# LanceZPF/loongx

Hardware: AMD Instinct MI355X
Metric: edited images/s @512x512, 28-step Flux denoise (higher is better)
Workload: dtype bf16

## Files before the change

### loongx_amd/csrc/rowops.hip

```cpp
#include "common.h"
#include <type_traits>

namespace {

struct LnLora { const uint16_t* A; float* T; int R, ldt, row0, rows; };

template <int NCH, bool LM = false, bool F16 = false>
__global__ __launch_bounds__(256, 3) void ln_modulate_kernel(const float* __restrict__ X, int ldx, const LnSegs segs, int mod_ld,
                                                          uint16_t* __restrict__ Y, int ldy, int M, int D, float eps, const LnLora lo = LnLora{},
                                                          int* __restrict__ f16_ovf = nullptr) {
  constexpr int RS = NCH * 256 + 32;
  __shared__ __attribute__((aligned(16))) uint16_t rows_s[LM ? 4 * RS : 8];
  __shared__ f32x4 red_s[LM ? 4 * 64 : 1];
  const int wave = threadIdx.x >> 6;
  const int row_l = blockIdx.x * 4 + wave;
  if constexpr (!LM) {
    if (row_l >= M) return;
  }
  const bool valid = row_l < M;
  auto phys = [&](int rl, int& sg_o, int& rin_o) {
    int sg = 0, acc_rows = 0;
    while (sg < segs.n - 1 && rl >= acc_rows + segs.n_rows[sg]) { acc_rows += segs.n_rows[sg]; ++sg; }
    sg_o = sg; rin_o = rl - acc_rows;
    return segs.row0[sg] + rin_o;
  };
  int sg, rin;
  const int row = phys(min(row_l, M - 1), sg, rin);
  bool wg_lora = false;
  if constexpr (LM) {
#pragma unroll
    for (int w = 0; w < 4; ++w) {
      const int rl = blockIdx.x * 4 + w;
      int s2, r2;
      const int pr = phys(min(rl, M - 1), s2, r2);
      wg_lora |= rl < M && pr >= lo.row0 && pr < lo.row0 + lo.rows;
    }
  }
  const float* shift = segs.shift[sg];
  const float* scale = segs.scale[sg];
  const int rows_per_batch = segs.rows_per_batch[sg];
  const int lane = threadIdx.x & 63;
  const float* xr = X + (size_t)row * ldx;
  f32x4 v[NCH];
  float s = 0.f;
#pragma unroll
  for (int i = 0; i < NCH; ++i) v[i] = *(const f32x4*)(xr + (i * 64 + lane) * 4);
  const int b = rin / rows_per_batch;
  const float* sh = shift + (size_t)b * mod_ld;
  const float* sc = scale + (size_t)b * mod_ld;
  f32x4 av[NCH], bv[NCH];
#pragma unroll
  for (int i = 0; i < NCH; ++i) {
    av[i] = *(const f32x4*)(sc + (i * 64 + lane) * 4);
    bv[i] = *(const f32x4*)(sh + (i * 64 + lane) * 4);
  }
#pragma unroll
  for (int i = 0; i < NCH; ++i) s += (v[i][0] + v[i][1]) + (v[i][2] + v[i][3]);
  const float mean = wave_total(s) / (float)D;
  float q = 0.f;
#pragma unroll
  for (int i = 0; i < NCH; ++i)
#pragma unroll
    for (int c = 0; c < 4; ++c) {
      const float d = v[i][c] - mean;
      q += d * d;
    }
  const float rstd = rsqrtf(wave_total(q) / (float)D + eps);
  uint16_t* yr = Y + (size_t)row * ldy;
  float f16_mx = 0.f;
#pragma unroll
  for (int i = 0; i < NCH; ++i) {
    const int col = (i * 64 + lane) * 4;
    float o[4];
#pragma unroll
    for (int c = 0; c < 4; ++c) o[c] = (v[i][c] - mean) * rstd * (1.0f + av[i][c]) + bv[i][c];
    u32x2 w;
    w[0] = pack_op16x2<F16>(o[0], o[1], f16_mx);
    w[1] = pack_op16x2<F16>(o[2], o[3], f16_mx);
    if (valid) *(u32x2*)(yr + col) = w;
    if constexpr (LM) {
      if (wg_lora) *(u32x2*)(rows_s + wave * RS + col) = w;
    }
  }
  if constexpr (LM) {
    if (wg_lora) {
      constexpr int NS = 2 * NCH, NB = NS >= 8 ? NS / 2 : NS;
      const int l15 = lane & 15, kq = lane >> 4;
      const uint16_t* ap = lo.A + (size_t)min(l15, lo.R - 1) * D + kq * 8;
      __builtin_amdgcn_sched_barrier(0);
      bf16x8 af[NB];
#pragma unroll
      for (int u = 0; u < NB; ++u) af[u] = *(const bf16x8*)(ap + (4 * u + wave) * 32);
      __syncthreads();
      f32x4 acc = {0.f, 0.f, 0.f, 0.f};
      const uint16_t* xp = rows_s + (l15 & 3) * RS + kq * 8;
      const bf16x8 zero = {};
#pragma unroll
      for (int u0 = 0; u0 < NS; u0 += NB) {
        if (u0 > 0) {
#pragma unroll
          for (int u = 0; u < NB; ++u) af[u] = *(const bf16x8*)(ap + (4 * (u0 + u) + wave) * 32);
        }
#pragma unroll
        for (int u = 0; u < NB; ++u) {
          bf16x8 xf = *(const bf16x8*)(xp + (4 * (u0 + u) + wave) * 32);
          xf = l15 < 4 ? xf : zero;
          if constexpr (F16) acc = __builtin_amdgcn_mfma_f32_16x16x32_f16(__builtin_bit_cast(f16x8, af[u]), __builtin_bit_cast(f16x8, xf), acc, 0, 0, 0);
          else acc = __builtin_amdgcn_mfma_f32_16x16x32_bf16(af[u], xf, acc, 0, 0, 0);
        }
      }
      red_s[wave * 64 + lane] = acc;
      __syncthreads();
      if (threadIdx.x < 64) {
        const int m = threadIdx.x >> 4, r = threadIdx.x & 15;
        const float* rp = (const float*)red_s + (m + 16 * (r >> 2)) * 4 + (r & 3);
        const float t = ((rp[0] + rp[256]) + rp[512]) + rp[768];
        const int rl = blockIdx.x * 4 + m;
        int s2, r2;
        const int pr = phys(min(rl, M - 1), s2, r2);
        if (rl < M && r < lo.R && pr >= lo.row0 && pr < lo.row0 + lo.rows) lo.T[(size_t)(pr - lo.row0) * lo.ldt + r] = t;
      }
    }
  }
  if constexpr (F16) report_f16_overflow(f16_mx, f16_ovf);
}

template <bool F16 = false>
__global__ __launch_bounds__(256) void ln_modulate_generic(const float* __restrict__ X, int ldx, const LnSegs segs, int mod_ld,
                                                           uint16_t* __restrict__ Y, int ldy, int M, int D, float eps, int* __restrict__ f16_ovf = nullptr) {
  int row = blockIdx.x * 4 + (threadIdx.x >> 6);
  if (row >= M) return;
  int sg = 0, acc_rows = 0;
  while (sg < segs.n - 1 && row >= acc_rows + segs.n_rows[sg]) { acc_rows += segs.n_rows[sg]; ++sg; }
  const int rin = row - acc_rows;
  row = segs.row0[sg] + rin;
  const float* shift = segs.shift[sg];
  const float* scale = segs.scale[sg];
  const int rows_per_batch = segs.rows_per_batch[sg];
  const int lane = threadIdx.x & 63;
  const float* xr = X + (size_t)row * ldx;
  float s = 0.f;
  for (int c = lane * 4; c < D; c += 256) {
    const f32x4 v = *(const f32x4*)(xr + c);
    s += (v[0] + v[1]) + (v[2] + v[3]);
  }
  const float mean = wave_sum(s) / (float)D;
  float q = 0.f;
  for (int c = lane * 4; c < D; c += 256) {
    const f32x4 v = *(const f32x4*)(xr + c);
#pragma unroll
    for (int k = 0; k < 4; ++k) q += (v[k] - mean) * (v[k] - mean);
  }
  const float rstd = rsqrtf(wave_sum(q) / (float)D + eps);
  const int b = rin / rows_per_batch;
  const float* sh = shift + (size_t)b * mod_ld;
  const float* sc = scale + (size_t)b * mod_ld;
  uint16_t* yr = Y + (size_t)row * ldy;
  float f16_mx = 0.f;
  for (int c = lane * 4; c < D; c += 256) {
    const f32x4 v = *(const f32x4*)(xr + c);
    const f32x4 a = *(const f32x4*)(sc + c);
    const f32x4 bsh = *(const f32x4*)(sh + c);
    float o[4];
#pragma unroll
    for (int k = 0; k < 4; ++k) o[k] = (v[k] - mean) * rstd * (1.0f + a[k]) + bsh[k];
    u32x2 w;
    w[0] = pack_op16x2<F16>(o[0], o[1], f16_mx);
    w[1] = pack_op16x2<F16>(o[2], o[3], f16_mx);
    *(u32x2*)(yr + c) = w;
  }
  if constexpr (F16) report_f16_overflow(f16_mx, f16_ovf);
}

__device__ __forceinline__ int vt_interleave(int key) {
  return (key & ~15) | (((key >> 2) & 1) << 3) | (((key >> 3) & 1) << 2) | (key & 3);
}

struct QkvSegs {
  int n;
  int row0[3], rows_per_batch[3], vt_pos0[3], tile0[4];
  const float* wq[3]; const float* wk[3]; const float* cos_tab[3]; const float* sin_tab[3];
};

__device__ __forceinline__ void unpack16x8(const u32x4 raw, float* x, bool in_f16) {
#pragma unroll
  for (int i = 0; i < 4; ++i) {
    if (in_f16) {
      x[2 * i] = (float)__builtin_bit_cast(_Float16, (uint16_t)(raw[i] & 0xffffu));
      x[2 * i + 1] = (float)__builtin_bit_cast(_Float16, (uint16_t)(raw[i] >> 16));
    } else {
      x[2 * i] = __uint_as_float(raw[i] << 16);
      x[2 * i + 1] = __uint_as_float(raw[i] & 0xffff0000u);
    }
  }
}
__device__ __forceinline__ u32x4 f16x8_to_bf16x8(const u32x4 raw) {
  float x[8];
  unpack16x8(raw, x, true);
  u32x4 o;
#pragma unroll
  for (int i = 0; i < 4; ++i) o[i] = pack_bf16x2(x[2 * i], x[2 * i + 1]);
  return o;
}

template <bool FAST, bool IN_F16 = false, bool KIMG = false>
__global__ __launch_bounds__(256) void qkv_prep_kernel(uint16_t* __restrict__ QKV, int ld, int q_col, int k_col, int v_col,
                                                       const QkvSegs segs, float eps, uint16_t* __restrict__ VT, int vt_ld, int H,
                                                       uint16_t* __restrict__ K2, int ldk2, int k2_col) {
  __shared__ uint16_t vt_s[64][128 + 8];
  int sg = 0;
  while (sg < segs.n - 1 && (int)blockIdx.x >= segs.tile0[sg + 1]) ++sg;
  const int p0 = ((int)blockIdx.x - segs.tile0[sg]) * 64;
  const int row0 = segs.row0[sg], rows_per_batch = segs.rows_per_batch[sg], vt_pos0 = segs.vt_pos0[sg];
  const float* __restrict__ wq = segs.wq[sg];
  const float* __restrict__ wk = segs.wk[sg];
  const float* __restrict__ cos_tab = segs.cos_tab[sg];
  const float* __restrict__ sin_tab = segs.sin_tab[sg];
  const int h = blockIdx.y;
  const int b = blockIdx.z;
  const int tid = threadIdx.x;
  const int sub = tid & 15;
  const int rloc = tid >> 4;
  const size_t rbase = (size_t)row0 + (size_t)b * rows_per_batch;
  if constexpr (FAST) {
    const f32x4 wq0 = *(const f32x4*)(wq + sub * 8), wq1 = *(const f32x4*)(wq + sub * 8 + 4);
    const f32x4 wk0 = *(const f32x4*)(wk + sub * 8), wk1 = *(const f32x4*)(wk + sub * 8 + 4);
#pragma unroll 1
    for (int half = 0; half < 2; ++half) {
      uint16_t* rowp[2];
      uint16_t* kdst[2];
      bool valid[2];
      u32x4 raw[2][3];
      f32x4 cs[2][4];
#pragma unroll
      for (int u = 0; u < 2; ++u) {
        const int p = p0 + (half * 2 + u) * 16 + rloc;
        valid[u] = p < rows_per_batch;
        const int pc = valid[u] ? p : 0;
        rowp[u] = QKV + (rbase + pc) * ld + h * 128 + sub * 8;
        kdst[u] = KIMG ? K2 + (rbase + pc) * ldk2 + k2_col + h * 128 + sub * 8 : rowp[u] + k_col;
        raw[u][0] = *(const u32x4*)(rowp[u] + q_col);
        raw[u][1] = *(const u32x4*)(rowp[u] + k_col);
        raw[u][2] = *(const u32x4*)(rowp[u] + v_col);
        const float* ct = cos_tab + (size_t)pc * 128 + sub * 8;
        const float* st = sin_tab + (size_t)pc * 128 + sub * 8;
        cs[u][0] = *(const f32x4*)ct; cs[u][1] = *(const f32x4*)(ct + 4);
        cs[u][2] = *(const f32x4*)st; cs[u][3] = *(const f32x4*)(st + 4);
      }
      __builtin_amdgcn_sched_barrier(0);
#pragma unroll
      for (int u = 0; u < 2; ++u) {
        u32x4 out[2];
#pragma unroll
        for (int which = 0; which < 2; ++which) {
          float x[8];
#pragma unroll
          for (int i = 0; i < 4; ++i) {
            x[2 * i] = __uint_as_float(raw[u][which][i] << 16);
            x[2 * i + 1] = __uint_as_float(raw[u][which][i] & 0xffff0000u);
          }
          float ss = 0.f;
#pragma unroll
          for (int i = 0; i < 8; ++i) ss += x[i] * x[i];
#pragma unroll
          for (int o = 8; o > 0; o >>= 1) ss += __shfl_xor(ss, o, 64);
          const float r = rsqrtf(ss * (1.0f / 128.0f) + eps);
          const f32x4 w0 = which ? wk0 : wq0, w1 = which ? wk1 : wq1;
#pragma unroll
          for (int i = 0; i < 4; ++i) { x[i] = x[i] * r * w0[i]; x[4 + i] = x[4 + i] * r * w1[i]; }
          float y[8];
#pragma unroll
          for (int i = 0; i < 4; ++i) {
            const float ce = i < 2 ? cs[u][0][2 * i] : cs[u][1][2 * i - 4], co = i < 2 ? cs[u][0][2 * i + 1] : cs[u][1][2 * i - 3];
            const float se = i < 2 ? cs[u][2][2 * i] : cs[u][3][2 * i - 4], so = i < 2 ? cs[u][2][2 * i + 1] : cs[u][3][2 * i - 3];
            y[2 * i] = x[2 * i] * ce - x[2 * i + 1] * se;
            y[2 * i + 1] = x[2 * i + 1] * co + x[2 * i] * so;
          }
#pragma unroll
          for (int i = 0; i < 4; ++i) out[which][i] = pack_bf16x2(y[2 * i], y[2 * i + 1]);
        }
        if (valid[u]) {
          *(u32x4*)(rowp[u] + q_col) = out[0];
          *(u32x4*)kdst[u] = out[1];
        }
        if (VT) *(u32x4*)&vt_s[(half * 2 + u) * 16 + rloc][sub * 8] = valid[u] ? raw[u][2] : u32x4{0u, 0u, 0u, 0u};
      }
    }
  } else {
#pragma unroll 1
  for (int pass = 0; pass < 4; ++pass) {
    const int p = p0 + pass * 16 + rloc;
    const bool valid = p < rows_per_batch;
    uint16_t* rowp = QKV + (rbase + (valid ? p : 0)) * ld + h * 128 + sub * 8;
    f32x4 c0 = {1.f, 1.f, 1.f, 1.f}, c1 = c0, s0 = {0.f, 0.f, 0.f, 0.f}, s1 = s0;
    if (cos_tab && valid) {
      const float* ct = cos_tab + (size_t)p * 128 + sub * 8;
      const float* st = sin_tab + (size_t)p * 128 + sub * 8;
      c0 = *(const f32x4*)ct; c1 = *(const f32x4*)(ct + 4);
      s0 = *(const f32x4*)st; s1 = *(const f32x4*)(st + 4);
    }
#pragma unroll
    for (int which = 0; which < 2; ++which) {
      const float* wn = which ? wk : wq;
      uint16_t* ptr = rowp + (which ? k_col : q_col);
      uint16_t* dst = ptr;
      if constexpr (KIMG) {
        if (which) dst = K2 + (rbase + (valid ? p : 0)) * ldk2 + k2_col + h * 128 + sub * 8;
      }
      u32x4 raw = {0u, 0u, 0u, 0u};
      if (valid) raw = *(const u32x4*)ptr;
      float x[8];
      unpack16x8(raw, x, IN_F16);
      if (wn) {
        float ss = 0.f;
#pragma unroll
        for (int i = 0; i < 8; ++i) ss += x[i] * x[i];
#pragma unroll
        for (int o = 8; o > 0; o >>= 1) ss += __shfl_xor(ss, o, 64);
        const float r = rsqrtf(ss * (1.0f / 128.0f) + eps);
        const f32x4 w0 = *(const f32x4*)(wn + sub * 8), w1 = *(const f32x4*)(wn + sub * 8 + 4);
#pragma unroll
        for (int i = 0; i < 4; ++i) { x[i] = x[i] * r * w0[i]; x[4 + i] = x[4 + i] * r * w1[i]; }
      }
      float y[8];
#pragma unroll
      for (int i = 0; i < 4; ++i) {
        const float ce = i < 2 ? c0[2 * i] : c1[2 * i - 4], co = i < 2 ? c0[2 * i + 1] : c1[2 * i - 3];
        const float se = i < 2 ? s0[2 * i] : s1[2 * i - 4], so = i < 2 ? s0[2 * i + 1] : s1[2 * i - 3];
        y[2 * i] = x[2 * i] * ce - x[2 * i + 1] * se;
        y[2 * i + 1] = x[2 * i + 1] * co + x[2 * i] * so;
      }
      if (valid) {
        u32x4 o;
#pragma unroll
        for (int i = 0; i < 4; ++i) o[i] = pack_bf16x2(y[2 * i], y[2 * i + 1]);
        *(u32x4*)dst = o;
      }
    }
    if (VT) {
      u32x4 raw = {0u, 0u, 0u, 0u};
      if (valid) raw = *(const u32x4*)(rowp + v_col);
      *(u32x4*)&vt_s[pass * 16 + rloc][sub * 8] = IN_F16 ? f16x8_to_bf16x8(raw) : raw;
    }
  }
  }
  if (!VT) return;
  __syncthreads();
  uint16_t* vtb = VT + ((size_t)(b * H + h) * 128) * vt_ld + vt_pos0 + p0;
  for (int item = tid; item < 128 * 8; item += 256) {
    const int d = item >> 3, g = item & 7;
    uint16_t e[8];
#pragma unroll
    for (int i = 0; i < 8; ++i) e[i] = vt_s[vt_interleave(g * 8 + i)][d];
    u32x4 o;
#pragma unroll
    for (int i = 0; i < 4; ++i) o[i] = (uint32_t)e[2 * i] | ((uint32_t)e[2 * i + 1] << 16);
    *(u32x4*)(vtb + (size_t)d * vt_ld + g * 8) = o;
  }
}

__device__ __forceinline__ float clamp_e4m3(float x) { return fminf(fmaxf(x, -448.f), 448.f); }
__device__ __forceinline__ uint32_t pack_fp8x4(float a, float b, float c, float d) {
  int w = __builtin_amdgcn_cvt_pk_fp8_f32(clamp_e4m3(a), clamp_e4m3(b), 0, false);
  w = __builtin_amdgcn_cvt_pk_fp8_f32(clamp_e4m3(c), clamp_e4m3(d), w, true);
  return (uint32_t)w;
}
__device__ __forceinline__ int vt8_key(int j) {
  const int g = j >> 5, p = j & 31;
  return (p >> 4) * 32 + 8 * ((p & 15) >> 2) + 4 * g + (p & 3);
}

template <bool IN_F16>
__global__ __launch_bounds__(256) void qkv_prep_fp8_kernel(const uint16_t* __restrict__ QKV, int ld, int q_col, int k_col, int v_col,
                                                           const QkvSegs segs, float eps, uint8_t* __restrict__ Q8,
                                                           uint8_t* __restrict__ K8, int ld8, uint8_t* __restrict__ VT8, int vt_ld,
                                                           int H, float q_scale, float k_scale, float v_scale) {
  __shared__ uint16_t vt_s[64][128 + 8];
  int sg = 0;
  while (sg < segs.n - 1 && (int)blockIdx.x >= segs.tile0[sg + 1]) ++sg;
  const int p0 = ((int)blockIdx.x - segs.tile0[sg]) * 64;
  const int row0 = segs.row0[sg], rows_per_batch = segs.rows_per_batch[sg], vt_pos0 = segs.vt_pos0[sg];
  const float* __restrict__ wq = segs.wq[sg];
  const float* __restrict__ wk = segs.wk[sg];
  const float* __restrict__ cos_tab = segs.cos_tab[sg];
  const float* __restrict__ sin_tab = segs.sin_tab[sg];
  const int h = blockIdx.y;
  const int b = blockIdx.z;
  const int tid = threadIdx.x;
  const int sub = tid & 15;
  const int rloc = tid >> 4;
  const size_t rbase = (size_t)row0 + (size_t)b * rows_per_batch;
#pragma unroll 1
  for (int pass = 0; pass < 4; ++pass) {
    const int p = p0 + pass * 16 + rloc;
    const bool valid = p < rows_per_batch;
    const size_t grow = rbase + (valid ? p : 0);
    const uint16_t* rowp = QKV + grow * ld + h * 128 + sub * 8;
    f32x4 c0 = {1.f, 1.f, 1.f, 1.f}, c1 = c0, s0 = {0.f, 0.f, 0.f, 0.f}, s1 = s0;
    if (cos_tab && valid) {
      const float* ct = cos_tab + (size_t)p * 128 + sub * 8;
      const float* st = sin_tab + (size_t)p * 128 + sub * 8;
      c0 = *(const f32x4*)ct; c1 = *(const f32x4*)(ct + 4);
      s0 = *(const f32x4*)st; s1 = *(const f32x4*)(st + 4);
    }
#pragma unroll
    for (int which = 0; which < 2; ++which) {
      const float* wn = which ? wk : wq;
      u32x4 raw = {0u, 0u, 0u, 0u};
      if (valid) raw = *(const u32x4*)(rowp + (which ? k_col : q_col));
      float x[8];
      unpack16x8(raw, x, IN_F16);
      if (wn) {
        float ss = 0.f;
#pragma unroll
        for (int i = 0; i < 8; ++i) ss += x[i] * x[i];
#pragma unroll
        for (int o = 8; o > 0; o >>= 1) ss += __shfl_xor(ss, o, 64);
        const float r = rsqrtf(ss * (1.0f / 128.0f) + eps);
        const f32x4 w0 = *(const f32x4*)(wn + sub * 8), w1 = *(const f32x4*)(wn + sub * 8 + 4);
#pragma unroll
        for (int i = 0; i < 4; ++i) { x[i] = x[i] * r * w0[i]; x[4 + i] = x[4 + i] * r * w1[i]; }
      }
      float y[8];
#pragma unroll
      for (int i = 0; i < 4; ++i) {
        const float ce = i < 2 ? c0[2 * i] : c1[2 * i - 4], co = i < 2 ? c0[2 * i + 1] : c1[2 * i - 3];
        const float se = i < 2 ? s0[2 * i] : s1[2 * i - 4], so = i < 2 ? s0[2 * i + 1] : s1[2 * i - 3];
        y[2 * i] = x[2 * i] * ce - x[2 * i + 1] * se;
        y[2 * i + 1] = x[2 * i + 1] * co + x[2 * i] * so;
      }
      if (valid) {
        const float sc = which ? k_scale : q_scale;
        u32x2 o;
        o[0] = pack_fp8x4(y[0] * sc, y[1] * sc, y[2] * sc, y[3] * sc);
        o[1] = pack_fp8x4(y[4] * sc, y[5] * sc, y[6] * sc, y[7] * sc);
        *(u32x2*)((which ? K8 : Q8) + grow * ld8 + h * 128 + sub * 8) = o;
      }
    }
    u32x4 raw = {0u, 0u, 0u, 0u};
    if (valid) raw = *(const u32x4*)(rowp + v_col);
    *(u32x4*)&vt_s[pass * 16 + rloc][sub * 8] = IN_F16 ? f16x8_to_bf16x8(raw) : raw;
  }
  __syncthreads();
  uint8_t* vtb = VT8 + ((size_t)(b * H + h) * 128) * vt_ld + vt_pos0 + p0;
  for (int item = tid; item < 128 * 4; item += 256) {
    const int d = item >> 2, c = item & 3;
    float e[16];
#pragma unroll
    for (int i = 0; i < 16; ++i) e[i] = __uint_as_float((uint32_t)vt_s[vt8_key(c * 16 + i)][d] << 16) * v_scale;
    u32x4 o;
#pragma unroll
    for (int i = 0; i < 4; ++i) o[i] = pack_fp8x4(e[4 * i], e[4 * i + 1], e[4 * i + 2], e[4 * i + 3]);
    *(u32x4*)(vtb + (size_t)d * vt_ld + c * 16) = o;
  }
}

struct LoraTerms {
  const uint16_t* X[4];
  const uint16_t* A[4];
  int ldx[4];
  int n;
};

template <bool F16 = false>
__global__ __launch_bounds__(512) void lora_down_mfma_kernel(const LoraTerms terms, float* __restrict__ T, int ldt, int M, int K, int R, int Ks,
                                                             int split_stride) {
  __shared__ f32x4 red[8][64];
  const int lane = threadIdx.x & 63, wave = threadIdx.x >> 6;
  const int m0 = blockIdx.x * 16;
  const int term = terms.n > 0 ? (int)blockIdx.y : 0;
  const uint16_t* __restrict__ X = terms.X[term];
  const uint16_t* __restrict__ A = terms.A[term];
  const int ldx = terms.ldx[term];
  const int kbeg = terms.n > 0 ? 0 : blockIdx.y * Ks, kend = terms.n > 0 ? K : min(K, kbeg + Ks);
  T += (size_t)blockIdx.y * split_stride;
  const int l15 = lane & 15, kq = lane >> 4;
  const uint16_t* xp = X + (size_t)min(m0 + l15, M - 1) * ldx + kq * 8;
  const uint16_t* ap = A + (size_t)min(l15, R - 1) * K + kq * 8;
  f32x4 acc = {0.f, 0.f, 0.f, 0.f};
  int k = kbeg + wave * 32;
  const bf16x8 zero = {};
  auto batch = [&](auto n_) {
    constexpr int NS = decltype(n_)::value;
    bf16x8 af[NS], xf[NS];
#pragma unroll
    for (int u = 0; u < NS; ++u) {
      const bool in = k + u * 256 < kend;
      af[u] = in ? *(const bf16x8*)(ap + k + u * 256) : zero;
      xf[u] = in ? *(const bf16x8*)(xp + k + u * 256) : zero;
    }
#pragma unroll
    for (int u = 0; u < NS; ++u) {
      if constexpr (F16) acc = __builtin_amdgcn_mfma_f32_16x16x32_f16(__builtin_bit_cast(f16x8, af[u]), __builtin_bit_cast(f16x8, xf[u]), acc, 0, 0, 0);
      else acc = __builtin_amdgcn_mfma_f32_16x16x32_bf16(af[u], xf[u], acc, 0, 0, 0);
    }
    k += NS * 256;
  };
  const int nsteps = k < kend ? (kend - k + 255) / 256 : 0;
  if (nsteps <= 4) batch(std::integral_constant<int, 4>{});
  else if (nsteps <= 8) batch(std::integral_constant<int, 8>{});
  else
    while (k < kend) batch(std::integral_constant<int, 16>{});
  red[wave][lane] = acc;
  __syncthreads();
  if (wave == 0) {
#pragma unroll
    for (int w = 1; w < 8; ++w) {
      const f32x4 o = red[w][lane];
      acc[0] += o[0]; acc[1] += o[1]; acc[2] += o[2]; acc[3] += o[3];
    }
    const int m = m0 + l15, r0 = 4 * kq;
    if (m < M && r0 < R) {
      float* tp = T + (size_t)m * ldt + r0;
      if (r0 + 4 <= R && (ldt & 3) == 0) *(f32x4*)tp = acc;
      else
        for (int j = 0; j < 4 && r0 + j < R; ++j) tp[j] = acc[j];
    }
  }
}

template <bool F16>
__global__ __launch_bounds__(512) void lora_down_wide_kernel(const uint16_t* __restrict__ X, int ldx, const uint16_t* __restrict__ A,
                                                             float* __restrict__ T, int ldt, int M, int K, int R, int Ks, int split_stride) {
  __shared__ f32x4 red[8][4][64];
  const int lane = threadIdx.x & 63, wave = threadIdx.x >> 6;
  const int m0 = blockIdx.x * 16, rz0 = blockIdx.z * 64;
  const int nt = min(4, (R - rz0 + 15) / 16);
  const int kbeg = blockIdx.y * Ks, kend = min(K, kbeg + Ks);
  T += (size_t)blockIdx.y * split_stride;
  const int l15 = lane & 15, kq = lane >> 4;
  const uint16_t* xp = X + (size_t)min(m0 + l15, M - 1) * ldx + kq * 8;
  const uint16_t* ap[4];
#pragma unroll
  for (int t = 0; t < 4; ++t) ap[t] = A + (size_t)min(rz0 + t * 16 + l15, R - 1) * K + kq * 8;
  f32x4 acc[4];
#pragma unroll
  for (int t = 0; t < 4; ++t) acc[t] = f32x4{0.f, 0.f, 0.f, 0.f};
  int k = kbeg + wave * 32;
  const bf16x8 zero = {};
  auto batch = [&](auto n_) {
    constexpr int NS = decltype(n_)::value;
    bf16x8 af[NS][4], xf[NS];
#pragma unroll
    for (int u = 0; u < NS; ++u) {
      const bool in = k + u * 256 < kend;
      xf[u] = in ? *(const bf16x8*)(xp + k + u * 256) : zero;
#pragma unroll
      for (int t = 0; t < 4; ++t) af[u][t] = (in && t < nt) ? *(const bf16x8*)(ap[t] + k + u * 256) : zero;
    }
#pragma unroll
    for (int u = 0; u < NS; ++u)
#pragma unroll
      for (int t = 0; t < 4; ++t)
        if (t < nt) {
          if constexpr (F16) acc[t] = __builtin_amdgcn_mfma_f32_16x16x32_f16(__builtin_bit_cast(f16x8, af[u][t]), __builtin_bit_cast(f16x8, xf[u]), acc[t], 0, 0, 0);
          else acc[t] = __builtin_amdgcn_mfma_f32_16x16x32_bf16(af[u][t], xf[u], acc[t], 0, 0, 0);
        }
    k += NS * 256;
  };
  const int nsteps = k < kend ? (kend - k + 255) / 256 : 0;
  if (nsteps <= 4) batch(std::integral_constant<int, 4>{});
  else
    while (k < kend) batch(std::integral_constant<int, 8>{});
#pragma unroll
  for (int t = 0; t < 4; ++t) red[wave][t][lane] = acc[t];
  __syncthreads();
  if (wave < nt) {
    f32x4 s = red[0][wave][lane];
#pragma unroll
    for (int w = 1; w < 8; ++w) {
      const f32x4 o = red[w][wave][lane];
      s[0] += o[0]; s[1] += o[1]; s[2] += o[2]; s[3] += o[3];
    }
    const int m = m0 + l15, r0 = rz0 + 16 * wave + 4 * kq;
    if (m < M && r0 < R) {
      float* tp = T + (size_t)m * ldt + r0;
      if (r0 + 4 <= R && (ldt & 3) == 0) *(f32x4*)tp = s;
      else
        for (int j = 0; j < 4 && r0 + j < R; ++j) tp[j] = s[j];
    }
  }
}

__device__ __forceinline__ float silu(float x) { return x / (1.0f + __expf(-x)); }

__global__ __launch_bounds__(256) void linear_skinny_kernel(const float* __restrict__ X, int ldx, const uint16_t* __restrict__ W,
                                                            int ldw, const float* __restrict__ bias, float* __restrict__ Y,
                                                            int ldy, int M, int N, int K, int act_in, int act_out, int accumulate) {
  const int wave = threadIdx.x >> 6, lane = threadIdx.x & 63;
  const int n0 = (blockIdx.x * 4 + wave) * 4;
  if (n0 >= N) return;
  const uint16_t* wr[4];
#pragma unroll
  for (int c = 0; c < 4; ++c) wr[c] = W + (size_t)min(n0 + c, N - 1) * ldw;
  for (int mb = 0; mb < M; mb += 4) {
    float acc[4][4];
#pragma unroll
    for (int i = 0; i < 4; ++i)
#pragma unroll
      for (int c = 0; c < 4; ++c) acc[i][c] = 0.f;
    for (int k = lane * 8; k < K; k += 512) {
      float wv[4][8];
#pragma unroll
      for (int c = 0; c < 4; ++c) {
        const u32x4 raw = *(const u32x4*)(wr[c] + k);
#pragma unroll
        for (int j = 0; j < 4; ++j) { wv[c][2 * j] = __uint_as_float(raw[j] << 16); wv[c][2 * j + 1] = __uint_as_float(raw[j] & 0xffff0000u); }
      }
#pragma unroll
      for (int i = 0; i < 4; ++i) {
        if (mb + i < M) {
          const float* xp = X + (size_t)(mb + i) * ldx + k;
          const f32x4 x0 = *(const f32x4*)xp, x1 = *(const f32x4*)(xp + 4);
          float xv[8] = {x0[0], x0[1], x0[2], x0[3], x1[0], x1[1], x1[2], x1[3]};
          if (act_in == 1) {
#pragma unroll
            for (int j = 0; j < 8; ++j) xv[j] = silu(xv[j]);
          }
#pragma unroll
          for (int c = 0; c < 4; ++c)
#pragma unroll
            for (int j = 0; j < 8; ++j) acc[i][c] = fmaf(xv[j], wv[c][j], acc[i][c]);
        }
      }
    }
#pragma unroll
    for (int i = 0; i < 4; ++i)
#pragma unroll
      for (int c = 0; c < 4; ++c) {
        float s = wave_sum(acc[i][c]);
        if (lane == 0 && mb + i < M && n0 + c < N) {
          if (bias) s += bias[n0 + c];
          if (act_out == 1) s = silu(s);
          float* yp = Y + (size_t)(mb + i) * ldy + n0 + c;
          *yp = accumulate ? (*yp + s) : s;
        }
      }
  }
}

__global__ void timestep_embed_kernel(const float* __restrict__ t, float* __restrict__ out, int B, int dim) {
  const int i = blockIdx.x * blockDim.x + threadIdx.x;
  const int half = dim / 2;
  if (i >= B * half) return;
  const int b = i / half, j = i % half;
  const float f = expf(-9.210340371976184f * (float)j / (float)half);
  const float a = t[b] * f;
  out[(size_t)b * dim + j] = cosf(a);
  out[(size_t)b * dim + half + j] = sinf(a);
}

__global__ void euler_kernel(float* __restrict__ x, const void* __restrict__ v, int v_bf16, float ds, size_t n) {
  const size_t stride = (size_t)gridDim.x * blockDim.x;
  for (size_t i = (size_t)blockIdx.x * blockDim.x + threadIdx.x; i < n; i += stride) {
    const float vv = v_bf16 ? bf16_to_f32(((const uint16_t*)v)[i]) : ((const float*)v)[i];
    x[i] = fmaf(ds, vv, x[i]);
  }
}

__global__ void convert_kernel(void* __restrict__ dst, int dst_bf16, const void* __restrict__ src, int src_bf16, size_t n) {
  const size_t stride = (size_t)gridDim.x * blockDim.x;
  for (size_t i = (size_t)blockIdx.x * blockDim.x + threadIdx.x; i < n; i += stride) {
    const float v = src_bf16 ? bf16_to_f32(((const uint16_t*)src)[i]) : ((const float*)src)[i];
    if (dst_bf16 == 2) {
      float mx = 0.f;
      ((uint16_t*)dst)[i] = (uint16_t)(pack_f16x2_sat(v, 0.f, mx) & 0xffffu);
    } else if (dst_bf16) ((uint16_t*)dst)[i] = f32_to_bf16(v);
    else ((float*)dst)[i] = v;
  }
}

}

static int ln_launch(const char* name, const float* X, int ldx, const lx_ln_seg* seg, int n_seg, int mod_ld, void* Y, int ldy, int D, float eps,
                     void* stream, const LnLora* lora = nullptr, bool f16 = false, int* f16_ovf = nullptr) {
  LX_CHECK_ARG(seg && n_seg >= 1 && n_seg <= 3, "%s: 1..3 segments", name);
  if (f16) LX_CHECK_ARG(((uintptr_t)f16_ovf & 3) == 0, "%s: f16_ovf must be 4-byte aligned", name);
  LnSegs segs;
  const int M = lx_ln_segs("lx_ln_modulate", seg, n_seg, segs);
  if (M < 0) return M;
  LX_CHECK_ARG(X && Y, "lx_ln_modulate: NULL operand");
  LX_CHECK_ARG(D > 0 && D % 4 == 0 && D <= 16384, "lx_ln_modulate: D=%d must be a multiple of 4 and <= 16384", D);
  LX_CHECK_ARG(ldx % 4 == 0 && ldy % 4 == 0 && mod_ld % 4 == 0, "lx_ln_modulate: ldx/ldy/mod_ld must be multiples of 4");
  LX_CHECK_ARG(((uintptr_t)X & 15) == 0 && ((uintptr_t)Y & 7) == 0, "lx_ln_modulate: misaligned operand");
  if (lora) {
    LX_CHECK_ARG(D == 3072 || D == 256, "lx_ln_modulate_lora_segs: the fused down-projection exists for D = 3072 and 256 (D=%d): use lx_lora_down", D);
    LX_CHECK_ARG(lora->A && lora->T && lora->R >= 1 && lora->R <= 16 && lora->ldt >= lora->R && lora->rows > 0 && lora->row0 >= 0,
                 "lx_ln_modulate_lora_segs: bad adapter arguments (R=%d)", lora->R);
    LX_CHECK_ARG(((uintptr_t)lora->A & 15) == 0, "lx_ln_modulate_lora_segs: Adown must be 16-byte aligned");
  }
  const LnLora lo = lora ? *lora : LnLora{};
  auto launch = [&](auto kernel, auto... tail) {
    hipLaunchKernelGGL(kernel, dim3((M + 3) / 4), dim3(256), 0, (hipStream_t)stream, X, ldx, segs, mod_ld, (uint16_t*)Y, ldy, M, D, eps, tail...);
  };
  auto dispatch = [&](auto lm, auto h) {
    constexpr bool LM = decltype(lm)::value, F16 = decltype(h)::value;
    if (D == 3072) launch(ln_modulate_kernel<12, LM, F16>, lo, f16_ovf);
    else if (D == 256) launch(ln_modulate_kernel<1, LM, F16>, lo, f16_ovf);
    else if constexpr (!LM) launch(ln_modulate_generic<F16>, f16_ovf);
  };
  if (lora && f16) dispatch(std::true_type{}, std::true_type{});
  else if (lora) dispatch(std::true_type{}, std::false_type{});
  else if (f16) dispatch(std::false_type{}, std::true_type{});
  else dispatch(std::false_type{}, std::false_type{});
  LX_LAUNCH_CHECK(lora ? "lx_ln_modulate_lora_segs" : f16 ? "lx_ln_modulate_f16_segs" : "lx_ln_modulate");
  return LX_OK;
}

extern "C" int lx_ln_modulate(const float* X, int ldx, const float* shift, const float* scale, int mod_ld, void* Y, int ldy,
                              int M, int D, int rows_per_batch, float eps, void* stream) {
  LX_CHECK_ARG(M > 0, "lx_ln_modulate: M must be > 0");
  const lx_ln_seg one = {0, M, rows_per_batch, 0, shift, scale};
  return ln_launch("lx_ln_modulate", X, ldx, &one, 1, mod_ld, Y, ldy, D, eps, stream);
}

extern "C" int lx_ln_modulate_segs(const float* X, int ldx, const lx_ln_seg* seg, int n_seg, int mod_ld, void* Y, int ldy, int D,
                                   float eps, void* stream) {
  return ln_launch("lx_ln_modulate_segs", X, ldx, seg, n_seg, mod_ld, Y, ldy, D, eps, stream);
}

extern "C" int lx_ln_modulate_f16_segs(const float* X, int ldx, const lx_ln_seg* seg, int n_seg, int mod_ld, void* Y, int ldy, int D,
                                       float eps, int32_t* f16_ovf, void* stream) {
  return ln_launch("lx_ln_modulate_f16_segs", X, ldx, seg, n_seg, mod_ld, Y, ldy, D, eps, stream, nullptr, true, (int*)f16_ovf);
}

extern "C" int lx_ln_modulate_lora_f16_segs(const float* X, int ldx, const lx_ln_seg* seg, int n_seg, int mod_ld, void* Y, int ldy, int D,
                                            float eps, const void* Adown, int R, float* T, int ldt, int lora_row0, int lora_rows,
                                            int32_t* f16_ovf, void* stream) {
  const LnLora lo{(const uint16_t*)Adown, T, R, ldt, lora_row0, lora_rows};
  return ln_launch("lx_ln_modulate_lora_f16_segs", X, ldx, seg, n_seg, mod_ld, Y, ldy, D, eps, stream, &lo, true, (int*)f16_ovf);
}

extern "C" int lx_ln_modulate_lora_segs(const float* X, int ldx, const lx_ln_seg* seg, int n_seg, int mod_ld, void* Y, int ldy, int D,
                                        float eps, const void* Adown, int R, float* T, int ldt, int lora_row0, int lora_rows, void* stream) {
  const LnLora lo{(const uint16_t*)Adown, T, R, ldt, lora_row0, lora_rows};
  return ln_launch("lx_ln_modulate_lora_segs", X, ldx, seg, n_seg, mod_ld, Y, ldy, D, eps, stream, &lo);
}

static int qkv_launch(void* QKV, int ld, int q_col, int k_col, int v_col, const lx_qkv_seg* seg, int n_seg, int n_batches, int H, float eps,
                      void* VT, int vt_ld, void* stream, bool in_f16 = false) {
  LX_CHECK_ARG(seg && n_seg >= 1 && n_seg <= 3, "lx_qkv_prep_segs: 1..3 segments");
  LX_CHECK_ARG(QKV && n_batches > 0 && H > 0, "lx_qkv_prep: bad arguments");
  LX_CHECK_ARG(ld % 8 == 0 && q_col % 8 == 0 && k_col % 8 == 0 && v_col % 8 == 0, "lx_qkv_prep: ld and column offsets must be multiples of 8");
  if (VT) LX_CHECK_ARG(vt_ld % 64 == 0, "lx_qkv_prep: vt_ld must be a multiple of 64");
  QkvSegs segs;
  const int t = lx_qkv_segs("lx_qkv_prep", seg, n_seg, VT ? LX_VT_POS0_MULT64 : LX_VT_POS0_ANY, segs, segs.vt_pos0);
  if (t < 0) return t;
  bool fast = true;
  for (int i = 0; i < segs.n; ++i) fast = fast && segs.wq[i] && segs.wk[i] && segs.cos_tab[i];
  auto launch = [&](auto kernel) {
    hipLaunchKernelGGL(kernel, dim3(t, H, n_batches), dim3(256), 0, (hipStream_t)stream, (uint16_t*)QKV, ld, q_col, k_col, v_col, segs, eps,
                       (uint16_t*)VT, vt_ld, H, (uint16_t*)nullptr, 0, 0);
  };
  if (in_f16) launch(qkv_prep_kernel<false, true>);
  else if (fast) launch(qkv_prep_kernel<true>);
  else launch(qkv_prep_kernel<false>);
  LX_LAUNCH_CHECK("lx_qkv_prep");
  return LX_OK;
}

extern "C" int lx_qkv_prep(void* QKV, int ld, int q_col, int k_col, int v_col, int row0, int n_rows, int rows_per_batch, int H,
                           const float* wq, const float* wk, float eps, const float* cos_tab, const float* sin_tab, void* VT,
                           int vt_ld, int vt_pos0, void* stream) {
  LX_CHECK_ARG(n_rows > 0 && rows_per_batch > 0 && n_rows % rows_per_batch == 0, "lx_qkv_prep: n_rows=%d must be a multiple of rows_per_batch=%d", n_rows, rows_per_batch);
  const lx_qkv_seg one = {row0, rows_per_batch, vt_pos0, 0, wq, wk, cos_tab, sin_tab};
  return qkv_launch(QKV, ld, q_col, k_col, v_col, &one, 1, n_rows / rows_per_batch, H, eps, VT, vt_ld, stream);
}

extern "C" int lx_qkv_prep_segs(void* QKV, int ld, int q_col, int k_col, int v_col, const lx_qkv_seg* seg, int n_seg, int n_batches,
                                int H, float eps, void* VT, int vt_ld, void* stream) {
  return qkv_launch(QKV, ld, q_col, k_col, v_col, seg, n_seg, n_batches, H, eps, VT, vt_ld, stream);
}

extern "C" int lx_qkv_prep_f16in_segs(void* QKV, int ld, int q_col, int k_col, int v_col, const lx_qkv_seg* seg, int n_seg, int n_batches,
                                      int H, float eps, void* VT, int vt_ld, void* stream) {
  return qkv_launch(QKV, ld, q_col, k_col, v_col, seg, n_seg, n_batches, H, eps, VT, vt_ld, stream, true);
}

static int qkv_kv_launch(const char* fn, bool in_f16, void* QKV, int ld, int q_col, int k_col, int v_col, const lx_qkv_seg* seg, int n_seg,
                         int n_batches, int H, float eps, void* K2, int ldk2, int k2_col, void* VT, int vt_ld, void* stream) {
  LX_CHECK_ARG(seg && n_seg >= 1 && n_seg <= 3, "%s: 1..3 segments", fn);
  LX_CHECK_ARG(QKV && K2 && VT && n_batches > 0 && H > 0, "%s: bad arguments", fn);
  LX_CHECK_ARG(ld % 8 == 0 && q_col % 8 == 0 && k_col % 8 == 0 && v_col % 8 == 0 && ((uintptr_t)QKV & 15) == 0,
               "%s: ld and column offsets must be multiples of 8, QKV 16-byte aligned", fn);
  LX_CHECK_ARG(ldk2 % 8 == 0 && k2_col % 8 == 0 && k2_col >= 0 && ldk2 >= k2_col + H * 128 && ((uintptr_t)K2 & 15) == 0,
               "%s: ldk2=%d / k2_col=%d must be multiples of 8 with k2_col + H*128 <= ldk2, K2 16-byte aligned", fn, ldk2, k2_col);
  LX_CHECK_ARG(vt_ld % 64 == 0 && ((uintptr_t)VT & 15) == 0, "%s: vt_ld must be a multiple of 64, VT 16-byte aligned", fn);
  QkvSegs segs;
  const int t = lx_qkv_segs(fn, seg, n_seg, LX_VT_POS0_MULT64_NONNEG, segs, segs.vt_pos0);
  if (t < 0) return t;
  for (int i = 0; i < n_seg; ++i) {
    const long long vt_end = (long long)seg[i].vt_pos0 + (seg[i].rows_per_batch + 63) / 64 * 64;
    LX_CHECK_ARG(vt_end <= vt_ld, "%s: segment %d's V^T tiles end at %lld > vt_ld=%d", fn, i, vt_end, vt_ld);
  }
  bool fast = true;
  for (int i = 0; i < segs.n; ++i) fast = fast && segs.wq[i] && segs.wk[i] && segs.cos_tab[i];
  auto launch = [&](auto kernel) {
    hipLaunchKernelGGL(kernel, dim3(t, H, n_batches), dim3(256), 0, (hipStream_t)stream, (uint16_t*)QKV, ld, q_col, k_col, v_col, segs, eps,
                       (uint16_t*)VT, vt_ld, H, (uint16_t*)K2, ldk2, k2_col);
  };
  if (in_f16) launch(qkv_prep_kernel<false, true, true>);
  else if (fast) launch(qkv_prep_kernel<true, false, true>);
  else launch(qkv_prep_kernel<false, false, true>);
  LX_LAUNCH_CHECK(fn);
  return LX_OK;
}

extern "C" int lx_qkv_prep_kv_segs(void* QKV, int ld, int q_col, int k_col, int v_col, const lx_qkv_seg* seg, int n_seg, int n_batches,
                                   int H, float eps, void* K2, int ldk2, int k2_col, void* VT, int vt_ld, void* stream) {
  return qkv_kv_launch("lx_qkv_prep_kv_segs", false, QKV, ld, q_col, k_col, v_col, seg, n_seg, n_batches, H, eps, K2, ldk2, k2_col, VT, vt_ld, stream);
}

extern "C" int lx_qkv_prep_kv_f16in_segs(void* QKV, int ld, int q_col, int k_col, int v_col, const lx_qkv_seg* seg, int n_seg, int n_batches,
                                         int H, float eps, void* K2, int ldk2, int k2_col, void* VT, int vt_ld, void* stream) {
  return qkv_kv_launch("lx_qkv_prep_kv_f16in_segs", true, QKV, ld, q_col, k_col, v_col, seg, n_seg, n_batches, H, eps, K2, ldk2, k2_col, VT, vt_ld,
                       stream);
}

static int qkv_fp8_segs_launch(bool in_f16, const void* QKV, int ld, int q_col, int k_col, int v_col, const lx_qkv_seg* seg, int n_seg,
                               int n_batches, int H, float eps, void* Q8, void* K8, int ld8, void* VT8, int vt8_ld,
                               float q_scale, float k_scale, float v_scale, void* stream) {
  LX_CHECK_ARG(seg && n_seg >= 1 && n_seg <= 3, "lx_qkv_prep_fp8_segs: 1..3 segments");
  LX_CHECK_ARG(QKV && Q8 && K8 && VT8 && n_batches > 0 && H > 0, "lx_qkv_prep_fp8_segs: bad arguments");
  LX_CHECK_ARG(ld % 8 == 0 && q_col % 8 == 0 && k_col % 8 == 0 && v_col % 8 == 0, "lx_qkv_prep_fp8_segs: ld and column offsets must be multiples of 8");
  LX_CHECK_ARG(ld8 % 16 == 0 && vt8_ld % 64 == 0, "lx_qkv_prep_fp8_segs: ld8 %% 16 and vt8_ld %% 64 required");
  LX_CHECK_ARG(q_scale > 0.f && k_scale > 0.f && v_scale > 0.f, "lx_qkv_prep_fp8_segs: scales must be positive");
  QkvSegs segs;
  const int t = lx_qkv_segs("lx_qkv_prep_fp8_segs", seg, n_seg, LX_VT_POS0_MULT64, segs, segs.vt_pos0);
  if (t < 0) return t;
  auto launch = [&](auto kernel) {
    hipLaunchKernelGGL(kernel, dim3(t, H, n_batches), dim3(256), 0, (hipStream_t)stream, (const uint16_t*)QKV, ld, q_col, k_col, v_col, segs, eps,
                       (uint8_t*)Q8, (uint8_t*)K8, ld8, (uint8_t*)VT8, vt8_ld, H, q_scale, k_scale, v_scale);
  };
  if (in_f16) launch(qkv_prep_fp8_kernel<true>);
  else launch(qkv_prep_fp8_kernel<false>);
  LX_LAUNCH_CHECK("lx_qkv_prep_fp8_segs");
  return LX_OK;
}

extern "C" int lx_qkv_prep_fp8_segs(const void* QKV, int ld, int q_col, int k_col, int v_col, const lx_qkv_seg* seg, int n_seg,
                                    int n_batches, int H, float eps, void* Q8, void* K8, int ld8, void* VT8, int vt8_ld,
                                    float q_scale, float k_scale, float v_scale, void* stream) {
  return qkv_fp8_segs_launch(false, QKV, ld, q_col, k_col, v_col, seg, n_seg, n_batches, H, eps, Q8, K8, ld8, VT8, vt8_ld, q_scale, k_scale, v_scale,
                             stream);
}

extern "C" int lx_qkv_prep_fp8_f16in_segs(const void* QKV, int ld, int q_col, int k_col, int v_col, const lx_qkv_seg* seg, int n_seg,
                                          int n_batches, int H, float eps, void* Q8, void* K8, int ld8, void* VT8, int vt8_ld,
                                          float q_scale, float k_scale, float v_scale, void* stream) {
  return qkv_fp8_segs_launch(true, QKV, ld, q_col, k_col, v_col, seg, n_seg, n_batches, H, eps, Q8, K8, ld8, VT8, vt8_ld, q_scale, k_scale, v_scale,
                             stream);
}

static int lora_down_launch(const char* name, bool f16, const void* X, int ldx, const void* Adown, float* T, int ldt, int M, int K, int R, int n_split,
                            int split_stride, void* stream) {
  LX_CHECK_ARG(X && Adown && T && M > 0, "%s: NULL operand", name);
  LX_CHECK_ARG(R >= 1 && R <= 256, "%s: R=%d must be in [1,256]", name, R);
  LX_CHECK_ARG(K % 32 == 0 && ldx % 8 == 0 && ldt >= R, "%s: K %% 32, ldx %% 8 and ldt >= R required (K=%d)", name, K);
  LX_CHECK_ARG(((uintptr_t)X & 15) == 0 && ((uintptr_t)Adown & 15) == 0 && ((uintptr_t)T & 15) == 0, "%s: operands must be 16-byte aligned", name);
  LX_CHECK_ARG(n_split >= 1 && n_split <= 16 && (n_split == 1 || split_stride >= (M - 1) * ldt + R) && split_stride % 4 == 0,
               "%s: bad n_split=%d / split_stride=%d", name, n_split, split_stride);
  const int Ks = ((K / 32 + n_split - 1) / n_split) * 32;
  if (R > 16) {
    const dim3 grid((M + 15) / 16, n_split, (R + 63) / 64);
    if (f16) hipLaunchKernelGGL(lora_down_wide_kernel<true>, grid, dim3(512), 0, (hipStream_t)stream, (const uint16_t*)X, ldx, (const uint16_t*)Adown, T, ldt, M, K, R, Ks, split_stride);
    else hipLaunchKernelGGL(lora_down_wide_kernel<false>, grid, dim3(512), 0, (hipStream_t)stream, (const uint16_t*)X, ldx, (const uint16_t*)Adown, T, ldt, M, K, R, Ks, split_stride);
    LX_LAUNCH_CHECK(name);
    return LX_OK;
  }
  LoraTerms lt = {};
  lt.X[0] = (const uint16_t*)X; lt.A[0] = (const uint16_t*)Adown; lt.ldx[0] = ldx; lt.n = 0;
  if (f16) hipLaunchKernelGGL(lora_down_mfma_kernel<true>, dim3((M + 15) / 16, n_split), dim3(512), 0, (hipStream_t)stream, lt, T, ldt, M, K, R, Ks, split_stride);
  else hipLaunchKernelGGL(lora_down_mfma_kernel<false>, dim3((M + 15) / 16, n_split), dim3(512), 0, (hipStream_t)stream, lt, T, ldt, M, K, R, Ks, split_stride);
  LX_LAUNCH_CHECK(name);
  return LX_OK;
}

extern "C" int lx_lora_down(const void* X, int ldx, const void* Adown, float* T, int ldt, int M, int K, int R, int n_split,
                            int split_stride, void* stream) {
  return lora_down_launch("lx_lora_down", false, X, ldx, Adown, T, ldt, M, K, R, n_split, split_stride, stream);
}

extern "C" int lx_lora_down_f16(const void* X, int ldx, const void* Adown, float* T, int ldt, int M, int K, int R, int n_split,
                                int split_stride, void* stream) {
  return lora_down_launch("lx_lora_down_f16", true, X, ldx, Adown, T, ldt, M, K, R, n_split, split_stride, stream);
}

extern "C" int lx_lora_down_terms(const void* const* X, const int* ldx, const void* const* Adown, int n_terms, float* T, int ldt, int M, int K,
                                  int R, int slab_stride, void* stream) {
  LX_CHECK_ARG(X && ldx && Adown && T && M > 0 && n_terms >= 1 && n_terms <= 4, "lx_lora_down_terms: bad arguments (1..4 terms)");
  LX_CHECK_ARG(R >= 1 && R <= 16 && K % 32 == 0 && ldt >= R && ((uintptr_t)T & 15) == 0, "lx_lora_down_terms: R in [1,16], K %% 32, ldt >= R, T 16-byte aligned required");
  LX_CHECK_ARG((n_terms == 1 || slab_stride >= (M - 1) * ldt + R) && slab_stride % 4 == 0, "lx_lora_down_terms: bad slab_stride=%d", slab_stride);
  LoraTerms lt = {};
  lt.n = n_terms;
  for (int i = 0; i < n_terms; ++i) {
    LX_CHECK_ARG(X[i] && Adown[i] && ldx[i] % 8 == 0 && ((uintptr_t)X[i] & 15) == 0 && ((uintptr_t)Adown[i] & 15) == 0, "lx_lora_down_terms: term %d: NULL / misaligned operand or ldx %% 8", i);
    lt.X[i] = (const uint16_t*)X[i]; lt.A[i] = (const uint16_t*)Adown[i]; lt.ldx[i] = ldx[i];
  }
  hipLaunchKernelGGL(lora_down_mfma_kernel<false>, dim3((M + 15) / 16, n_terms), dim3(512), 0, (hipStream_t)stream, lt, T, ldt, M, K, R, K, slab_stride);
  LX_LAUNCH_CHECK("lx_lora_down_terms");
  return LX_OK;
}

extern "C" int lx_linear_skinny(const float* X, int ldx, const void* W, int ldw, const float* bias, float* Y, int ldy, int M, int N,
                                int K, int act_in, int act_out, int accumulate, void* stream) {
  LX_CHECK_ARG(X && W && Y, "lx_linear_skinny: NULL operand");
  LX_CHECK_ARG(M >= 1 && M <= 65536, "lx_linear_skinny: M=%d must be in [1,65536]", M);
  LX_CHECK_ARG(K % 8 == 0 && ldw % 8 == 0 && ldx % 4 == 0, "lx_linear_skinny: K %% 8, ldw %% 8, ldx %% 4 required (K=%d)", K);
  const dim3 grid((N + 15) / 16), block(256);
  hipLaunchKernelGGL(linear_skinny_kernel, grid, block, 0, (hipStream_t)stream, X, ldx, (const uint16_t*)W, ldw, bias, Y, ldy, M, N,
                     K, act_in, act_out, accumulate);
  LX_LAUNCH_CHECK("lx_linear_skinny");
  return LX_OK;
}

extern "C" int lx_timestep_embed(const float* t, float* out, int B, int dim, void* stream) {
  LX_CHECK_ARG(t && out && B > 0 && dim > 0 && dim % 2 == 0, "lx_timestep_embed: bad arguments");
  const int n = B * dim / 2;
  hipLaunchKernelGGL(timestep_embed_kernel, dim3((n + 255) / 256), dim3(256), 0, (hipStream_t)stream, t, out, B, dim);
  LX_LAUNCH_CHECK("lx_timestep_embed");
  return LX_OK;
}

extern "C" int lx_euler_step(float* x, const void* v, int v_is_bf16, float dsigma, size_t n, void* stream) {
  LX_CHECK_ARG(x && v, "lx_euler_step: NULL operand");
  if (n == 0) return LX_OK;
  const int grid = (int)((n + 255) / 256 < 2048 ? (n + 255) / 256 : 2048);
  hipLaunchKernelGGL(euler_kernel, dim3(grid), dim3(256), 0, (hipStream_t)stream, x, v, v_is_bf16, dsigma, n);
  LX_LAUNCH_CHECK("lx_euler_step");
  return LX_OK;
}

extern "C" int lx_convert(void* dst, int dst_bf16, const void* src, int src_bf16, size_t n, void* stream) {
  LX_CHECK_ARG(dst && src, "lx_convert: NULL operand");
  if (n == 0) return LX_OK;
  const int grid = (int)((n + 255) / 256 < 4096 ? (n + 255) / 256 : 4096);
  hipLaunchKernelGGL(convert_kernel, dim3(grid), dim3(256), 0, (hipStream_t)stream, dst, dst_bf16, src, src_bf16, n);
  LX_LAUNCH_CHECK("lx_convert");
  return LX_OK;
}

namespace {
__global__ void rope_table_kernel(const float* __restrict__ ids, int n_axes, int a0, int a1, int a2, double theta,
                                  float* __restrict__ cos_t, float* __restrict__ sin_t, int L) {
  const int dims[3] = {a0, a1, a2};
  const int total = a0 + a1 + a2;
  const int i = blockIdx.x * blockDim.x + threadIdx.x;
  if (i >= L * (total / 2)) return;
  const int p = i / (total / 2);
  int j = i % (total / 2), axis = 0, off = 0;
  while (axis < n_axes - 1 && j >= dims[axis] / 2) { j -= dims[axis] / 2; off += dims[axis]; ++axis; }
  const double freq = 1.0 / pow(theta, (double)(2 * j) / (double)dims[axis]);
  const double ang = (double)ids[(size_t)p * n_axes + axis] * freq;
  const float c = (float)cos(ang), s = (float)sin(ang);
  const size_t o = (size_t)p * total + off + 2 * j;
  cos_t[o] = c; cos_t[o + 1] = c;
  sin_t[o] = s; sin_t[o + 1] = s;
}
}

extern "C" int lx_rope_table(const float* ids, int L, int a0, int a1, int a2, double theta, float* cos_t, float* sin_t, void* stream) {
  LX_CHECK_ARG(ids && cos_t && sin_t && L > 0, "lx_rope_table: bad arguments");
  LX_CHECK_ARG(a0 > 0 && a1 > 0 && a2 > 0 && a0 % 2 == 0 && a1 % 2 == 0 && a2 % 2 == 0, "lx_rope_table: axes dims must be positive and even");
  const int n = L * (a0 + a1 + a2) / 2;
  hipLaunchKernelGGL(rope_table_kernel, dim3((n + 255) / 256), dim3(256), 0, (hipStream_t)stream, ids, 3, a0, a1, a2, theta, cos_t, sin_t, L);
  LX_LAUNCH_CHECK("lx_rope_table");
  return LX_OK;
}
```

Before: 1.039.

## Stage shared modulation vectors in LDS per workgroup in LayerNorm-modulate kernel

After: 1.042, median of 6. Within noise of the previous version (+0.3%).

```diff
diff --git a/loongx_amd/csrc/rowops.hip b/loongx_amd/csrc/rowops.hip
--- a/loongx_amd/csrc/rowops.hip
+++ b/loongx_amd/csrc/rowops.hip
@@ -5,54 +5,76 @@
 
 struct LnLora { const uint16_t* A; float* T; int R, ldt, row0, rows; };
 
-template <int NCH, bool LM = false, bool F16 = false>
-__global__ __launch_bounds__(256, 3) void ln_modulate_kernel(const float* __restrict__ X, int ldx, const LnSegs segs, int mod_ld,
-                                                          uint16_t* __restrict__ Y, int ldy, int M, int D, float eps, const LnLora lo = LnLora{},
-                                                          int* __restrict__ f16_ovf = nullptr) {
+template <int NCH, bool LM, bool F16, bool STAGE, typename Phys>
+__device__ __forceinline__ float ln_modulate_body(const float* __restrict__ X, int ldx, const LnSegs& segs, int mod_ld, uint16_t* __restrict__ Y,
+                                                 int ldy, int M, int D, float eps, const LnLora& lo, const Phys& phys,
+                                                 bool wg_lora, int sg0, int rin0, int b0, uint16_t* rows_s, f32x4* red_s, f32x4* mod_s) {
+#pragma clang fp contract(off)
   constexpr int RS = NCH * 256 + 32;
-  __shared__ __attribute__((aligned(16))) uint16_t rows_s[LM ? 4 * RS : 8];
-  __shared__ f32x4 red_s[LM ? 4 * 64 : 1];
+  constexpr int NV = NCH * 64;
   const int wave = threadIdx.x >> 6;
   const int row_l = blockIdx.x * 4 + wave;
-  if constexpr (!LM) {
-    if (row_l >= M) return;
-  }
-  const bool valid = row_l < M;
-  auto phys = [&](int rl, int& sg_o, int& rin_o) {
-    int sg = 0, acc_rows = 0;
-    while (sg < segs.n - 1 && rl >= acc_rows + segs.n_rows[sg]) { acc_rows += segs.n_rows[sg]; ++sg; }
-    sg_o = sg; rin_o = rl - acc_rows;
-    return segs.row0[sg] + rin_o;
-  };
-  int sg, rin;
-  const int row = phys(min(row_l, M - 1), sg, rin);
-  bool wg_lora = false;
-  if constexpr (LM) {
-#pragma unroll
-    for (int w = 0; w < 4; ++w) {
-      const int rl = blockIdx.x * 4 + w;
-      int s2, r2;
-      const int pr = phys(min(rl, M - 1), s2, r2);
-      wg_lora |= rl < M && pr >= lo.row0 && pr < lo.row0 + lo.rows;
-    }
-  }
-  const float* shift = segs.shift[sg];
-  const float* scale = segs.scale[sg];
-  const int rows_per_batch = segs.rows_per_batch[sg];
+  if constexpr (!LM && !STAGE) {
+    if (row_l >= M) return 0.f;
+  }
+  const bool valid = STAGE || row_l < M;
+  int sg = sg0, rin = rin0 + wave;
+  int row = segs.row0[sg0] + rin;
+  if constexpr (!STAGE) row = phys(min(row_l, M - 1), sg, rin);
   const int lane = threadIdx.x & 63;
   const float* xr = X + (size_t)row * ldx;
+  const int b = STAGE ? b0 : rin / segs.rows_per_batch[sg];
+  const float* sh = segs.shift[sg] + (size_t)b * mod_ld;
+  const float* sc = segs.scale[sg] + (size_t)b * mod_ld;
+  constexpr int NS = 2 * NCH, NB = NS >= 8 ? NS / 2 : NS;
+  const int l15 = lane & 15, kq = lane >> 4;
+  const uint16_t* ap = nullptr;
+  if constexpr (LM && STAGE) ap = lo.A + (size_t)min(l15, lo.R - 1) * D + kq * 8;
+  constexpr int NM = STAGE ? (NV + 255) / 256 : 1;
+  f32x4 ms[NM], mh[NM];
+  if constexpr (STAGE) {
+#pragma unroll
+    for (int j = 0; j < NM; ++j) {
+      const int c = j * 256 + (int)threadIdx.x;
+      if (NV % 256 == 0 || c < NV) {
+        ms[j] = *(const f32x4*)(sc + c * 4);
+        mh[j] = *(const f32x4*)(sh + c * 4);
+      }
+    }
+  }
   f32x4 v[NCH];
   float s = 0.f;
 #pragma unroll
   for (int i = 0; i < NCH; ++i) v[i] = *(const f32x4*)(xr + (i * 64 + lane) * 4);
-  const int b = rin / rows_per_batch;
-  const float* sh = shift + (size_t)b * mod_ld;
-  const float* sc = scale + (size_t)b * mod_ld;
-  f32x4 av[NCH], bv[NCH];
-#pragma unroll
-  for (int i = 0; i < NCH; ++i) {
-    av[i] = *(const f32x4*)(sc + (i * 64 + lane) * 4);
-    bv[i] = *(const f32x4*)(sh + (i * 64 + lane) * 4);
+  f32x4 av[STAGE ? 1 : NCH], bv[STAGE ? 1 : NCH];
+  bf16x8 af[LM ? NB : 1];
+  constexpr bool AF2 = STAGE && LM && !F16 && NS > NB;
+  static_assert(!AF2 || NB == NCH, "one second-batch fragment per row chunk");
+  bf16x8 af2[AF2 ? NB : 1];
+  if constexpr (STAGE) {
+    if constexpr (LM) {
+      if (wg_lora) {
+#pragma unroll
+        for (int u = 0; u < NB; ++u) af[u] = *(const bf16x8*)(ap + (4 * u + wave) * 32);
+      }
+    }
+#pragma unroll
+    for (int j = 0; j < NM; ++j) {
+      const int c = j * 256 + (int)threadIdx.x;
+      if (NV % 256 == 0 || c < NV) {
+        f32x4 a1;
+#pragma unroll
+        for (int k = 0; k < 4; ++k) a1[k] = 1.0f + ms[j][k];
+        mod_s[c] = a1;
+        mod_s[NV + c] = mh[j];
+      }
+    }
+  } else {
+#pragma unroll
+    for (int i = 0; i < NCH; ++i) {
+      av[i] = *(const f32x4*)(sc + (i * 64 + lane) * 4);
+      bv[i] = *(const f32x4*)(sh + (i * 64 + lane) * 4);
+    }
   }
 #pragma unroll
   for (int i = 0; i < NCH; ++i) s += (v[i][0] + v[i][1]) + (v[i][2] + v[i][3]);
@@ -63,17 +85,32 @@
 #pragma unroll
     for (int c = 0; c < 4; ++c) {
       const float d = v[i][c] - mean;
-      q += d * d;
+      if (F16 && NCH == 12 && i == 0 && c == 0) continue;
+      if (F16 && NCH == 12 && i == 0 && c == 1) {
+        const float d0 = v[0][0] - mean;
+        q = __builtin_fmaf(d0, d0, d * d);
+      } else if (F16 && NCH == 12 && i < NCH - 1) q = __builtin_fmaf(d, d, q);
+      else q += d * d;
     }
   const float rstd = rsqrtf(wave_total(q) / (float)D + eps);
   uint16_t* yr = Y + (size_t)row * ldy;
   float f16_mx = 0.f;
+  if constexpr (STAGE) __syncthreads();
 #pragma unroll
   for (int i = 0; i < NCH; ++i) {
     const int col = (i * 64 + lane) * 4;
+    f32x4 a1, bs;
+    if constexpr (STAGE) {
+      a1 = mod_s[i * 64 + lane];
+      bs = mod_s[NV + i * 64 + lane];
+    } else {
+#pragma unroll
+      for (int c = 0; c < 4; ++c) a1[c] = 1.0f + av[i][c];
+      bs = bv[i];
+    }
     float o[4];
 #pragma unroll
-    for (int c = 0; c < 4; ++c) o[c] = (v[i][c] - mean) * rstd * (1.0f + av[i][c]) + bv[i][c];
+    for (int c = 0; c < 4; ++c) o[c] = __builtin_fmaf((v[i][c] - mean) * rstd, a1[c], bs[c]);
     u32x2 w;
     w[0] = pack_op16x2<F16>(o[0], o[1], f16_mx);
     w[1] = pack_op16x2<F16>(o[2], o[3], f16_mx);
@@ -81,16 +118,18 @@
     if constexpr (LM) {
       if (wg_lora) *(u32x2*)(rows_s + wave * RS + col) = w;
     }
+    if constexpr (AF2) {
+      if (wg_lora) af2[i] = *(const bf16x8*)(ap + (4 * (NB + i) + wave) * 32);
+    }
   }
   if constexpr (LM) {
     if (wg_lora) {
-      constexpr int NS = 2 * NCH, NB = NS >= 8 ? NS / 2 : NS;
-      const int l15 = lane & 15, kq = lane >> 4;
-      const uint16_t* ap = lo.A + (size_t)min(l15, lo.R - 1) * D + kq * 8;
-      __builtin_amdgcn_sched_barrier(0);
-      bf16x8 af[NB];
-#pragma unroll
-      for (int u = 0; u < NB; ++u) af[u] = *(const bf16x8*)(ap + (4 * u + wave) * 32);
+      if constexpr (!STAGE) {
+        ap = lo.A + (size_t)min(l15, lo.R - 1) * D + kq * 8;
+        __builtin_amdgcn_sched_barrier(0);
+#pragma unroll
+        for (int u = 0; u < NB; ++u) af[u] = *(const bf16x8*)(ap + (4 * u + wave) * 32);
+      }
       __syncthreads();
       f32x4 acc = {0.f, 0.f, 0.f, 0.f};
       const uint16_t* xp = rows_s + (l15 & 3) * RS + kq * 8;
@@ -99,7 +138,7 @@
       for (int u0 = 0; u0 < NS; u0 += NB) {
         if (u0 > 0) {
 #pragma unroll
-          for (int u = 0; u < NB; ++u) af[u] = *(const bf16x8*)(ap + (4 * (u0 + u) + wave) * 32);
+          for (int u = 0; u < NB; ++u) af[u] = AF2 ? af2[u] : *(const bf16x8*)(ap + (4 * (u0 + u) + wave) * 32);
         }
 #pragma unroll
         for (int u = 0; u < NB; ++u) {
@@ -122,6 +161,44 @@
       }
     }
   }
+  return f16_mx;
+}
+
+template <int NCH, bool LM = false, bool F16 = false>
+__global__ __launch_bounds__(256, 3) void ln_modulate_kernel(const float* __restrict__ X, int ldx, const LnSegs segs, int mod_ld,
+                                                          uint16_t* __restrict__ Y, int ldy, int M, int D, float eps, int stage,
+                                                          const LnLora lo = LnLora{}, int* __restrict__ f16_ovf = nullptr) {
+  __shared__ __attribute__((aligned(16))) uint16_t rows_s[LM ? 4 * (NCH * 256 + 32) : 8];
+  __shared__ f32x4 red_s[LM ? 4 * 64 : 1];
+  __shared__ f32x4 mod_s[2 * NCH * 64];
+  auto phys = [&](int rl, int& sg_o, int& rin_o) {
+    int sg = 0, acc_rows = 0;
+    while (sg < segs.n - 1 && rl >= acc_rows + segs.n_rows[sg]) { acc_rows += segs.n_rows[sg]; ++sg; }
+    sg_o = sg; rin_o = rl - acc_rows;
+    return segs.row0[sg] + rin_o;
+  };
+  bool wg_lora = false, wg_stage = false;
+  int sg0 = 0, rin0 = 0, b0 = 0;
+  if constexpr (LM) {
+#pragma unroll
+    for (int w = 0; w < 4; ++w) {
+      const int rl = blockIdx.x * 4 + w;
+      int s2, r2;
+      const int pr = phys(min(rl, M - 1), s2, r2);
+      wg_lora |= rl < M && pr >= lo.row0 && pr < lo.row0 + lo.rows;
+    }
+  }
+  if (stage != 0 && (int)blockIdx.x * 4 + 3 < M) {
+    int s3, r3;
+    phys(blockIdx.x * 4, sg0, rin0);
+    phys(blockIdx.x * 4 + 3, s3, r3);
+    const int rpb = segs.rows_per_batch[sg0];
+    b0 = rin0 / rpb;
+    wg_stage = s3 == sg0 && r3 / rpb == b0;
+  }
+  float f16_mx;
+  if (wg_stage) f16_mx = ln_modulate_body<NCH, LM, F16, true>(X, ldx, segs, mod_ld, Y, ldy, M, D, eps, lo, phys, wg_lora, sg0, rin0, b0, rows_s, red_s, mod_s);
+  else f16_mx = ln_modulate_body<NCH, LM, F16, false>(X, ldx, segs, mod_ld, Y, ldy, M, D, eps, lo, phys, wg_lora, sg0, rin0, b0, rows_s, red_s, mod_s);
   if constexpr (F16) report_f16_overflow(f16_mx, f16_ovf);
 }
 
@@ -690,13 +767,15 @@
     LX_CHECK_ARG(((uintptr_t)lora->A & 15) == 0, "lx_ln_modulate_lora_segs: Adown must be 16-byte aligned");
   }
   const LnLora lo = lora ? *lora : LnLora{};
+  const char* e = getenv("LX_LN_STAGE");
+  const int stage = e ? atoi(e) != 0 : 1;
   auto launch = [&](auto kernel, auto... tail) {
     hipLaunchKernelGGL(kernel, dim3((M + 3) / 4), dim3(256), 0, (hipStream_t)stream, X, ldx, segs, mod_ld, (uint16_t*)Y, ldy, M, D, eps, tail...);
   };
   auto dispatch = [&](auto lm, auto h) {
     constexpr bool LM = decltype(lm)::value, F16 = decltype(h)::value;
-    if (D == 3072) launch(ln_modulate_kernel<12, LM, F16>, lo, f16_ovf);
-    else if (D == 256) launch(ln_modulate_kernel<1, LM, F16>, lo, f16_ovf);
+    if (D == 3072) launch(ln_modulate_kernel<12, LM, F16>, stage, lo, f16_ovf);
+    else if (D == 256) launch(ln_modulate_kernel<1, LM, F16>, stage, lo, f16_ovf);
     else if constexpr (!LM) launch(ln_modulate_generic<F16>, f16_ovf);
   };
   if (lora && f16) dispatch(std::true_type{}, std::true_type{});
```
